# REGRAGUIahmed/DGViT-Depth-Goal-Guided-Vision-Transformer-

Hardware: AMD Instinct MI355X
Metric: depth frames/sec through DGViT fwd+bwd, batch 512x84x84 (higher is better)
Workload: dtype f32

## Files before the change

### dgvit-depth-goal-guided-vision-transformer-_amd/_lib.py

```python
import ctypes
import os
from ctypes import POINTER, Structure, c_char_p, c_float, c_int, c_longlong, c_ulonglong, c_void_p

_HERE = os.path.dirname(os.path.abspath(__file__))
LIB_PATH = os.path.join(_HERE, "libdgvit_hip.so")
DIAG_LIB_PATH = os.path.join(_HERE, "libdgvit_hip_diag.so")


class DgvitError(RuntimeError):
    pass


class dgvit_config(Structure):
    _fields_ = [("image_h", c_int), ("image_w", c_int), ("patch_h", c_int), ("patch_w", c_int), ("dim", c_int),
                ("depth", c_int), ("heads", c_int), ("dim_head", c_int), ("mlp_dim", c_int), ("pool_mean", c_int), ("flags", c_int)]


FLAG_DENSE_LAST_BLOCK = 1
FLAG_WGRAD_OVERLAP = 2
FLAG_LONG_SEQUENCE = 4
MAPS_GOAL = 0
MAPS_ALL = 1


# ... 79 lines not shown
    "dgvit_got_backward_bf16_ev": (_I, [_CFG, _TABLE, _P, _TABLE, _P, _P, _P, _P, _LL, _P, _LL, _I, _F, _ULL, _P, _P, POINTER(dgvit_grad_events)]),
    "dgvit_got_backward_bf16_v2": (_I, [_CFG, _TABLE, _P, _TABLE, _P, _P, _P, _P, _P, _LL, _P, _LL, _I, _F, _ULL, _P, _P]),
    "dgvit_got_backward_bf16_v2_ev": (_I, [_CFG, _TABLE, _P, _TABLE, _P, _P, _P, _P, _P, _LL, _P, _LL, _I, _F, _ULL, _P, _P,
                                           POINTER(dgvit_grad_events)]),
    "dgvit_wgrad_bf16_scratch_floats": (_LL, [_I, _I, _I]),
    "dgvit_wgrad_bf16": (_I, [_P, _P, _P, _P, _P, _LL, _I, _I, _I, _P]),
    "dgvit_cast_f32_bf16": (_I, [_P, _P, _LL, _P]),
    "dgvit_gemm_bf16": (_I, [_I, _P, _I, _P, _I, _P, _I, _I, _I, _I, _P, _P, _I, _P, _I, _P, _I, _P]),
    "dgvit_layernorm_forward_bf16": (_I, [_P, _P, _P, _P, _P, _P, _I, _I, _P]),
    "dgvit_attention_forward_bf16": (_I, [_P, _P, _P, _I, _I, _I, _I, _P]),
    "dgvit_got_forward_maps": (_I, [_CFG, _TABLE, _P, _P, _P, _P, _I, _P, _LL, _I, _F, _F, _ULL, _P, _P]),
    "dgvit_got_forward_maps_bf16": (_I, [_CFG, _TABLE, _P, _P, _P, _P, _P, _I, _P, _LL, _I, _F, _ULL, _P, _P]),
    "dgvit_attention_probs": (_I, [_P, _P, _P, _I, _I, _I, _I, _I, _P]),
    "dgvit_attention_probs_bf16": (_I, [_P, _P, _P, _I, _I, _I, _I, _I, _P]),
    "dgvit_attention_backward_bf16": (_I, [_P, _P, _P, _P, _P, _P, _I, _I, _I, _I, _P]),
    "dgvit_profile_start": (_I, [_I]),
    "dgvit_profile_stop": (_I, [POINTER(ctypes.c_double), POINTER(ctypes.c_double), POINTER(c_longlong)]),
    "dgvit_profile_sampling": (_I, [_I]),
    "dgvit_profile_totals": (_I, [POINTER(ctypes.c_double), POINTER(c_longlong)]),
}
DIAG_SIGNATURES = {
    "dgvit_set_gemm_tile": (None, [_I]),
    "dgvit_set_grouped_reduce": (None, [_I]),
    "dgvit_set_gemm_split": (None, [_I]),
    "dgvit_set_gemm_lds_pad": (None, [_I]),
    "dgvit_set_ln_fusion": (None, [_I]),
    "dgvit_set_conv_gather": (None, [_I]),
    "dgvit_set_gemm_diagnostics": (None, [_I]),
    "dgvit_set_gemm_persistent": (None, [_I, _I]),
    "dgvit_gemm_persistent_launches": (ctypes.c_longlong, []),
    "dgvit_set_gemm_stamps": (None, [_P, _I]),
    "dgvit_set_small_batch_path": (None, [_I, _I]),
    "dgvit_set_block_path": (None, [_I, _I]),
    "dgvit_set_block_stamps": (None, [_P]),
    "dgvit_set_block_stamp_layer": (None, [_I]),
    "dgvit_set_gelu_grad_store": (None, [_I]),
    "dgvit_set_block_fuse": (None, [_I]),
    "dgvit_set_gemm_bf16_tile": (None, [_I]),
    "dgvit_set_gemm_bf16_group_m": (None, [_I]),
    "dgvit_set_gemm_bf16_l2_budget_kb": (None, [_I]),
    "dgvit_set_attention_bwd_single_pass": (None, [_I]),
    "dgvit_set_attention_single_query": (None, [_I]),
    "dgvit_set_attention_bf16_long": (None, [_I]),
    "dgvit_set_gemm_wgrad_slice_major": (None, [_I]),
    "dgvit_attention_forward_queries": (_I, [_P, _P, _P, _I, _I, _I, _I, _I, _P]),
    "dgvit_attention_backward_queries": (_I, [_P, _P, _P, _P, _P, _I, _I, _I, _I, _I, _P]),
# ... 60 lines not shown
```

### dgvit-depth-goal-guided-vision-transformer-_amd/csrc/diag_api.hip

```cpp
#define DGVIT_KNOB_DEFINE
#include "../../include/dgvit_hip_diag.h"
#include "schedule.h"

#ifndef DGVIT_DIAG
#error "diag_api.hip belongs to the diagnostic library only (-DDGVIT_DIAG)"
#endif

long long g_gemm_persist_launches = 0;

extern "C" void dgvit_set_gemm_tile(int tile) { g_gemm_tile_hint = tile; }
extern "C" void dgvit_set_grouped_reduce(int on) { g_group_reduce = on ? 1 : 0; }
extern "C" void dgvit_set_conv_gather(int on) { g_conv_gather = on ? 1 : 0; }
extern "C" void dgvit_set_ln_fusion(int on) { g_ln_fusion = on ? 1 : 0; }
extern "C" void dgvit_set_gemm_split(int on) { g_gemm_split = on ? 1 : 0; }
extern "C" void dgvit_set_gemm_stamps(long long* stamps, int workgroups) {
  g_gemm_stamps = stamps;
  g_gemm_stamp_capacity = stamps ? workgroups : 0;
}
extern "C" long long dgvit_gemm_persistent_launches(void) { return g_gemm_persist_launches; }
extern "C" void dgvit_set_gemm_persistent(int mode, int workgroups) {
  g_gemm_persist = mode < 0 ? 0 : (mode > 2 ? 2 : mode);
  g_gemm_persist_grid = workgroups > 0 ? workgroups : 0;
}
extern "C" void dgvit_set_gemm_diagnostics(int on) { g_gemm_diag = on & 0x3FFFFF; }
extern "C" void dgvit_set_gemm_lds_pad(int bytes) { g_gemm_lds_pad = bytes > 0 ? bytes : 0; }
extern "C" void dgvit_set_small_batch_path(int on, int max_rows) {
  g_small_path = on ? 1 : 0;
  if (max_rows > 0) g_small_path_max_rows = max_rows;
}
extern "C" void dgvit_set_block_path(int on, int max_rows) {
  g_block_path = on < 0 ? 0 : (on > 2 ? 2 : on);
  g_block_path_max_rows = max_rows > 0 ? max_rows : g_block_path_max_rows_default;
}
extern "C" void dgvit_set_block_stamps(long long* stamps) { g_block_stamps = stamps; }
// ... 20 lines not shown
```

### dgvit-depth-goal-guided-vision-transformer-_amd/csrc/encoder.hip

```cpp
#include <mutex>

#include "schedule.h"

namespace {
struct Side {
  hipStream_t stream = nullptr;
  hipEvent_t ring[32];
  unsigned next = 0;
  bool ready = false;
};
Side g_side;
std::mutex g_side_mu;

int side_init() {
  std::lock_guard<std::mutex> lk(g_side_mu);
  if (g_side.ready) return DGVIT_OK;
  if (hipStreamCreateWithFlags(&g_side.stream, hipStreamNonBlocking) != hipSuccess)
    return dgvit_set_error(DGVIT_ERR_HIP, "cannot create the helper stream");
  for (auto& e : g_side.ring)
    if (hipEventCreateWithFlags(&e, hipEventDisableTiming) != hipSuccess)
      return dgvit_set_error(DGVIT_ERR_HIP, "cannot create helper events");
  g_side.ready = true;
  return DGVIT_OK;
}
int chain(hipStream_t from, hipStream_t to) {
  hipEvent_t e = g_side.ring[g_side.next++ % 32];
  if (hipEventRecord(e, from) != hipSuccess || hipStreamWaitEvent(to, e, 0) != hipSuccess)
    return dgvit_set_error(DGVIT_ERR_HIP, "event fork/join failed");
  return DGVIT_OK;
}
}
// ... 386 lines not shown
  f.maps_rows = rows;
  return got_forward(f, img, goal, feat, ws_floats, batch, keep);
}

namespace {

struct Bwd {
  const dgvit_config* cfg;
  Dims d;
  Ws w;
  Bs s;
  const float* const* params;
  float* const* grads;
  const float* ws;
  float* scratch;
  SplitBuf sk;
  float lkeep;
  bool ldrop;
  unsigned long long seed;
  const unsigned long long* seed_dev;
  hipStream_t st;
  hipStream_t sw;
  const dgvit_grad_events* events;
  LayerDrop site(int layer, int s) const { return LayerDrop{lkeep, drop_tag(layer, s), seed, seed_dev}; }
  int fork() const { return sw == st ? DGVIT_OK : chain(st, sw); }
  int join() const { return sw == st ? DGVIT_OK : chain(sw, st); }
};

int backward_layer(const Bwd& b, int i) {
  const Dims& d = b.d;
  const Ws& w = b.w;
  const Bs& s = b.s;
  const float* ws = b.ws;
  float* scratch = b.scratch;
  const bool ldrop = b.ldrop;
  hipStream_t st = b.st, sw = b.sw;
  const SplitBuf& sk = b.sk;
  const int T = (int)d.T;
  float* dx = scratch + s.dxa;
  float* dx2 = scratch + s.dxb;
  float* dln = scratch + s.dln;
  float* dqkv = scratch + s.dqkv;
  float* dao = scratch + s.dao;
  float* dh1 = scratch + s.dh1;
  float* slabs = scratch + s.slabs;
  const float* const* lp = b.params + P_L0 + DGVIT_PARAMS_PER_LAYER * i;
  float* const* lg = b.grads + P_L0 + DGVIT_PARAMS_PER_LAYER * i;
  const float* lb = ws + w.layer0 + w.layer_stride * i;
  const float* xin = i == 0 ? ws + w.x0 : ws + w.layer0 + w.layer_stride * (i - 1) + w.xout;
  const bool last = !dense_last_block(b.cfg) && !d.pool_mean && i == d.L - 1;
  const int tok = last ? d.B : T, rs = last ? d.N : 1;
  ReduceGroup grp;
  reduce_group_init(grp);
  ReduceGroup* gq = g_group_reduce ? &grp : nullptr;
  const float* dff = dx;
  if (ldrop) {
    TRY(drop_rows(dx, (long long)rs * d.D, scratch + s.dm3, (long long)rs * d.D, nullptr, 0, tok, d.D, rs, b.site(i, DROP_FF), st));
    dff = scratch + s.dm3;
  }
  TRY(b.fork());
  TRY(wgrad(dff, rs * d.D, lb + w.a1, d.M, lg[L_FC2W], lg[L_FC2B], d.D, d.M, tok, slabs + s.sl_fc2, s.n_fc2, sw, gq));
  {
    GemmParams p = gp(dff, rs * d.D, lp[L_FC2W], d.M, dh1, d.M, tok, d.M, d.D);
    p.aux = lb + w.h1; p.ldaux = d.M;
    sk.attach(p);
    TRY(gemm_f32(GEMM_NN, g_gelu_grad_store || ldrop ? EPI_DMUL : EPI_DGELU, p, 1, st));
  }
  TRY(b.fork());
  TRY(wgrad(dh1, d.M, lb + w.ln2, rs * d.D, lg[L_FC1W], lg[L_FC1B], d.M, d.D, tok, slabs + s.sl_fc1, s.n_fc1, sw, gq));
  {
    GemmParams p = gp(dh1, d.M, lp[L_FC1W], d.D, dln, rs * d.D, tok, d.D, d.M);
    sk.attach(p);
    TRY(gemm_f32(GEMM_NN, EPI_STORE, p, 1, st));
  }
  if (last) HIP_TRY(hipMemsetAsync(dx2, 0, sizeof(float) * d.T * d.D, st));
  TRY(layernorm_bwd(dln, lb + w.xmid, lb + w.mean2, lb + w.rstd2, lp[L_LN2W], dx, dx2, lg[L_LN2W], lg[L_LN2B], scratch + s.part_ln2, tok, d.D,
                    rs, st, gq));
  if (d.proj) {
    const float* dat = dx2;
    if (ldrop) {
      TRY(drop_rows(dx2, (long long)rs * d.D, scratch + s.dm1, (long long)rs * d.D, nullptr, 0, tok, d.D, rs, b.site(i, DROP_OUT), st));
      dat = scratch + s.dm1;
    }
    TRY(b.fork());
    TRY(wgrad(dat, rs * d.D, lb + w.ao, rs * d.I, lg[L_OUTW], lg[L_OUTB], d.D, d.I, tok, slabs + s.sl_out, s.n_out, sw, gq));
    GemmParams p = gp(dat, rs * d.D, lp[L_OUTW], d.I, dao, rs * d.I, tok, d.I, d.D);
    sk.attach(p);
    TRY(gemm_f32(GEMM_NN, EPI_STORE, p, 1, st));
  }
  const LayerDrop dr_attn = b.site(i, DROP_ATTN);
  if (d.tiled)
    TRY(attention_bwd_tiled(lb + w.qkv, lb + w.ao, d.proj ? dao : dx2, lb + w.lse, dqkv, scratch + s.delta, s.delta_floats, d.B, d.N, d.H,
                            d.dh, last ? 1 : d.N, st, ldrop ? &dr_attn : nullptr));
  else
    TRY(attention_bwd(lb + w.qkv, lb + w.ao, d.proj ? dao : dx2, lb + w.lse, dqkv, d.B, d.N, d.H, d.dh, last ? 1 : d.N, st,
                      ldrop ? &dr_attn : nullptr));
  TRY(b.fork());
  if (!last) {
    TRY(wgrad(dqkv, 3 * d.I, lb + w.ln1, d.D, lg[L_QKV], nullptr, 3 * d.I, d.D, T, slabs + s.sl_qkv, s.n_qkv, sw, gq));
    GemmParams p = gp(dqkv, 3 * d.I, lp[L_QKV], d.D, dln, d.D, T, d.D, 3 * d.I);
    sk.attach(p);
    TRY(gemm_f32(GEMM_NN, EPI_STORE, p, 1, st));
  } else {
    const long long nq_slabs = wgrad_scratch(d.I, d.D, tok);
    TRY(wgrad(dqkv, rs * 3 * d.I, lb + w.ln1, rs * d.D, lg[L_QKV], nullptr, d.I, d.D, tok, slabs + s.sl_qkv, nq_slabs, sw, gq));
    TRY(wgrad(dqkv + d.I, 3 * d.I, lb + w.ln1, d.D, lg[L_QKV] ? lg[L_QKV] + (long long)d.I * d.D : nullptr, nullptr, 2 * d.I, d.D, T,
              slabs + s.sl_qkv + nq_slabs, s.n_qkv - nq_slabs, sw, gq));
    GemmParams kv = gp(dqkv + d.I, 3 * d.I, lp[L_QKV] + (long long)d.I * d.D, d.D, dln, d.D, T, d.D, 2 * d.I);
    sk.attach(kv);
    TRY(gemm_f32(GEMM_NN, EPI_STORE, kv, 1, st));
    GemmParams q = gp(dqkv, rs * 3 * d.I, lp[L_QKV], d.D, dln, rs * d.D, tok, d.D, d.I);
    q.res = dln; q.ldr = rs * d.D;
    sk.attach(q);
    TRY(gemm_f32(GEMM_NN, EPI_STORE, q, 1, st));
  }
  TRY(b.join());
  TRY(layernorm_bwd(dln, xin, lb + w.mean1, lb + w.rstd1, lp[L_LN1W], dx2, dx, lg[L_LN1W], lg[L_LN1B], scratch + s.part_ln1, T, d.D, 1, st, gq));
  TRY(b.fork());
  TRY(reduce_group_flush(grp, sw));
  TRY(b.join());
  if (b.events) TRY(mark_ready(b.events->layer[i], st));
  return DGVIT_OK;
}

}

extern "C" int dgvit_got_backward(const dgvit_config* cfg, const float* const* params, float* const* grads, const float* dfeat,
                                  float* dgoal, const float* ws, long long ws_floats, float* scratch, long long scratch_floats,
                                  int batch, float keep, unsigned long long seed, const unsigned long long* seed_dev,
                                  void* stream) {
  return dgvit_got_backward_v2_ev(cfg, params, grads, dfeat, dgoal, ws, ws_floats, scratch, scratch_floats, batch, keep, 1.f, seed, seed_dev,
                                  stream, nullptr);
}

extern "C" int dgvit_got_backward_ev(const dgvit_config* cfg, const float* const* params, float* const* grads, const float* dfeat,
                                     float* dgoal, const float* ws, long long ws_floats, float* scratch, long long scratch_floats,
                                     int batch, float keep, unsigned long long seed, const unsigned long long* seed_dev,
                                     void* stream, const dgvit_grad_events* events) {
  return dgvit_got_backward_v2_ev(cfg, params, grads, dfeat, dgoal, ws, ws_floats, scratch, scratch_floats, batch, keep, 1.f, seed, seed_dev,
                                  stream, events);
}

extern "C" int dgvit_got_backward_v2(const dgvit_config* cfg, const float* const* params, float* const* grads, const float* dfeat,
// ... 5 lines not shown
}

extern "C" int dgvit_got_backward_v2_ev(const dgvit_config* cfg, const float* const* params, float* const* grads, const float* dfeat,
                                        float* dgoal, const float* ws, long long ws_floats, float* scratch, long long scratch_floats,
                                        int batch, float keep, float lkeep, unsigned long long seed, const unsigned long long* seed_dev,
                                        void* stream, const dgvit_grad_events* events) {
  return dgvit_got_backward_v3_ev(cfg, params, grads, dfeat, dgoal, nullptr, ws, ws_floats, scratch, scratch_floats, batch, keep, lkeep, seed,
                                  seed_dev, stream, events);
}

extern "C" int dgvit_got_backward_v3(const dgvit_config* cfg, const float* const* params, float* const* grads, const float* dfeat,
                                     float* dgoal, float* dimg, const float* ws, long long ws_floats, float* scratch, long long scratch_floats,
                                     int batch, float keep, float lkeep, unsigned long long seed, const unsigned long long* seed_dev,
                                     void* stream) {
  return dgvit_got_backward_v3_ev(cfg, params, grads, dfeat, dgoal, dimg, ws, ws_floats, scratch, scratch_floats, batch, keep, lkeep, seed,
                                  seed_dev, stream, nullptr);
}

extern "C" int dgvit_got_backward_v3_ev(const dgvit_config* cfg, const float* const* params, float* const* grads, const float* dfeat,
                                        float* dgoal, float* dimg, const float* ws, long long ws_floats, float* scratch, long long scratch_floats,
                                        int batch, float keep, float lkeep, unsigned long long seed, const unsigned long long* seed_dev,
                                        void* stream, const dgvit_grad_events* events) {
  hipStream_t st = (hipStream_t)stream;
  Bwd b = {cfg, {}, {}, {}, params, grads, ws, scratch, {}, lkeep, lkeep < 1.f, seed, seed_dev, st, st, events};
  const Dims& d = b.d;
  TRY(make_dims(cfg, batch, b.d));
  DGVIT_CHECK_ARG(params && grads && dfeat && ws && scratch, "dgvit_got_backward: null pointer");
  DGVIT_CHECK_ARG(keep > 0.f && keep <= 1.f, "dropout_keep must be in (0, 1]");
  DGVIT_CHECK_ARG(lkeep > 0.f && lkeep <= 1.f, "layer_dropout_keep must be in (0, 1]");
  TRY(check_events(events, cfg->depth));
  b.w = make_ws(d, 1);
  b.s = make_bs(d);
  const Ws& w = b.w;
  const Bs& s = b.s;
  if (ws_floats < w.total) return dgvit_set_error(DGVIT_ERR_WORKSPACE, "backward workspace %lld < %lld floats", ws_floats, w.total);
  if (scratch_floats < s.total) return dgvit_set_error(DGVIT_ERR_WORKSPACE, "backward scratch %lld < %lld floats", scratch_floats, s.total);
  const int np = P_L0 + DGVIT_PARAMS_PER_LAYER * d.L;
  for (int i = 0; i < np; ++i) DGVIT_CHECK_ARG(params[i] || no_projection_slot(d, i), "parameter %d is null", i);
  float* dx = scratch + s.dxa;
  float* dln = scratch + s.dln;
  float* part = scratch + s.part;

  if (s.sk_slab_floats > 0) {
    b.sk.counters = reinterpret_cast<int*>(scratch + s.sk_counters); b.sk.ncounters = (int)s.sk_ncounters;
    b.sk.slabs = scratch + s.sk_slabs; b.sk.slab_cap = s.sk_slab_floats;
    HIP_TRY(hipMemsetAsync(b.sk.counters, 0, sizeof(int) * s.sk_ncounters, st));
  }
  if (wgrad_overlap(cfg)) {
    TRY(side_init());
    b.sw = g_side.stream;
    TRY(chain(st, b.sw));
  }
  const float* xl = ws + w.layer0 + w.layer_stride * (d.L - 1) + w.xout;
  TRY(head_bwd(d, dfeat, xl, ws + w.pooled, params[P_RMS], grads[P_RMS], dx, dln, part, events, st));
  for (int i = d.L - 1; i >= 0; --i) TRY(backward_layer(b, i));
  return token_assembly_bwd(cfg, d, params, grads, dx, dgoal, dimg, dln, ws + w.patches, nullptr, nullptr, part, scratch + s.slabs,
                            s.slabs_floats, keep, seed, seed_dev, st);
}
```

### dgvit-depth-goal-guided-vision-transformer-_amd/csrc/kernels.h

```cpp
#pragma once
#include "common.h"

int layernorm_fwd(const float*, const float*, const float*, float*, float*, float*, int, int, float, int, hipStream_t);
int layernorm_bwd_blocks(int T);
int layernorm_bwd(const float*, const float*, const float*, const float*, const float*, const float*, float*, float*, float*,
                  float*, int, int, int, hipStream_t, ReduceGroup* grp = nullptr);
int rmsnorm_fwd(const float*, long long, const float*, float*, int, int, hipStream_t);
int rmsnorm_bwd_blocks(int B);
int rmsnorm_bwd(const float*, const float*, long long, const float*, float*, long long, float*, float*, int, int, hipStream_t);
int colsum_blocks(int T);
int colsum(const float*, long long, float*, float*, int, int, int, hipStream_t);
int attention_fwd(const float*, float*, float*, int, int, int, int, int, hipStream_t, const LayerDrop* drop = nullptr);
int attention_bwd(const float*, const float*, const float*, const float*, float*, int, int, int, int, int, hipStream_t,
                  const LayerDrop* drop = nullptr);
int attention_fwd_tiled(const float*, float*, float*, int, int, int, int, int, hipStream_t, const LayerDrop* drop = nullptr);
long long attention_bwd_tiled_scratch(int B, int N, int H);
int attention_bwd_tiled(const float*, const float*, const float*, const float*, float*, float*, long long, int, int, int, int, int,
                        hipStream_t, const LayerDrop* drop = nullptr);
int attention_probs(const float* qkv, const float* lse, float* probs, long long frame_stride, int B, int N, int H, int dh, int rows,
                    hipStream_t st);
int patchify(const float*, float*, int, int, int, int, int, hipStream_t);
int add_rows(const float*, long long, const float*, long long, float*, long long, long long, int, hipStream_t);
int goal_row(const float*, const float*, float*, int, int, int, hipStream_t);
int dropout_inplace(float*, long long, unsigned long long, const unsigned long long*, float, hipStream_t);
int drop_rows(const float* src, long long lds, float* dst, long long ldd, const float* res, long long ldr, long long rows, int width, int rs,
              const LayerDrop& drop, hipStream_t stream);
int relu_bwd(const float*, const float*, float*, long long, hipStream_t);
int adam_step(float*, const float*, float*, float*, long long, float, float, float, float, float, long long, const long long*,
              hipStream_t);
// ... 37 lines not shown
```

### dgvit-depth-goal-guided-vision-transformer-_amd/csrc/knobs.h

```cpp
#pragma once

#ifdef DGVIT_DIAG
#ifdef DGVIT_KNOB_DEFINE
#define DGVIT_KNOB(type, name, def) type name = def; constexpr type name##_default = def;
#else
#define DGVIT_KNOB(type, name, def) extern type name;
#endif
#define DGVIT_DIAG_ONLY(...) __VA_ARGS__
#define KNOB_IF(k) if (k)
#else
#define DGVIT_KNOB(type, name, def) static constexpr type name = def;
#define DGVIT_DIAG_ONLY(...)
#define KNOB_IF(k) if constexpr ((k) != 0)
#endif

DGVIT_KNOB(int, g_gemm_tile_hint, 0)
DGVIT_KNOB(int, g_gemm_split, 1)
DGVIT_KNOB(int, g_gemm_lds_pad, 0)
DGVIT_KNOB(int, g_gemm_persist, 0)
DGVIT_KNOB(int, g_gemm_persist_grid, 0)
DGVIT_KNOB(int, g_gemm_diag, 0)
DGVIT_KNOB(long long*, g_gemm_stamps, nullptr)
DGVIT_KNOB(int, g_gemm_stamp_capacity, 0)
DGVIT_KNOB(int, g_group_reduce, 1)
DGVIT_KNOB(int, g_ln_fusion, 1)
DGVIT_KNOB(int, g_conv_gather, 1)
DGVIT_KNOB(int, g_gelu_grad_store, 1)
DGVIT_KNOB(int, g_block_path, 1)
DGVIT_KNOB(int, g_block_fuse, 2)
DGVIT_KNOB(int, g_block_path_max_rows, 4160)
DGVIT_KNOB(long long*, g_block_stamps, nullptr)
DGVIT_KNOB(int, g_block_stamp_layer, -1)
DGVIT_KNOB(int, g_block_stamp_now, 1)
DGVIT_KNOB(int, g_small_path, 0)
DGVIT_KNOB(int, g_small_path_max_rows, 4160)
DGVIT_KNOB(int, g_gemm_bf16_tile_hint, 0)
DGVIT_KNOB(int, g_gemm_bf16_m16, 1)
DGVIT_KNOB(int, g_gemm_bf16_group_m, 8)
DGVIT_KNOB(int, g_gemm_bf16_l2_budget_kb, 2048)
DGVIT_KNOB(long long*, g_gemm_bf16_stamps, nullptr)
DGVIT_KNOB(int, g_attn_bwd64, 1)
DGVIT_KNOB(int, g_gemm_zfold, 1)
DGVIT_KNOB(int, g_attn_q1, 1)
DGVIT_KNOB(int, g_attn_bf16_long, 3)
#ifdef DGVIT_DIAG
extern long long g_gemm_persist_launches;
#endif
// ... 1 lines not shown
```

### dgvit-depth-goal-guided-vision-transformer-_amd/csrc/norm.hip

```cpp
#include "common.h"
#include "kernels.h"
#include "bf16.h"

namespace {

__device__ __forceinline__ float4 load4(const float* p) { return *reinterpret_cast<const float4*>(p); }
__device__ __forceinline__ float4 load4(const bf16_t* p) {
  const fx4 v = __builtin_convertvector(*reinterpret_cast<const bf16x4*>(p), fx4);
  return make_float4(v[0], v[1], v[2], v[3]);
}

__global__ void __launch_bounds__(256) layernorm_fwd_kernel(const float* __restrict__ x, const float* __restrict__ gamma,
                                                            const float* __restrict__ beta, float* __restrict__ y,
                                                            float* __restrict__ mean, float* __restrict__ rstd, int T, int D,
                                                            float eps, int rs) {
  const int lane = threadIdx.x & 63;
  const int row = blockIdx.x * 4 + (threadIdx.x >> 6);
  if (row >= T) return;
  const float* xr = x + (long long)row * rs * D;
  float s = 0.f;
  for (int c = lane * 4; c < D; c += 256) {
    const float4 v = *reinterpret_cast<const float4*>(xr + c);
    s += (v.x + v.y) + (v.z + v.w);
  }
// ... 8 lines not shown
  float* yr = y + (long long)row * rs * D;
  for (int c = lane * 4; c < D; c += 256) {
    const float4 v = *reinterpret_cast<const float4*>(xr + c);
    const float4 g = *reinterpret_cast<const float4*>(gamma + c);
    const float4 b = *reinterpret_cast<const float4*>(beta + c);
    float4 o;
    o.x = (v.x - mu) * rsd * g.x + b.x;
    o.y = (v.y - mu) * rsd * g.y + b.y;
    o.z = (v.z - mu) * rsd * g.z + b.z;
    o.w = (v.w - mu) * rsd * g.w + b.w;
    *reinterpret_cast<float4*>(yr + c) = o;
  }
  if (lane == 0) {
    mean[row] = mu;
    rstd[row] = rsd;
  }
}

template <int NCH, typename DYT>
__global__ void __launch_bounds__(256) layernorm_bwd_kernel(const DYT* __restrict__ dy, const float* __restrict__ x,
                                                            const float* __restrict__ mean, const float* __restrict__ rstd,
                                                            const float* __restrict__ gamma, const float* __restrict__ dres,
                                                            float* __restrict__ dx, bf16_t* __restrict__ dxb,
                                                            float* __restrict__ partial, int T, int D, int rs) {
  __shared__ float red[4][2][NCH * 256];
  const int lane = threadIdx.x & 63, wave = threadIdx.x >> 6;
  float4 ag[NCH], ab[NCH], gm[NCH];
#pragma unroll
  for (int i = 0; i < NCH; ++i) {
    ag[i] = make_float4(0.f, 0.f, 0.f, 0.f);
    ab[i] = ag[i];
    const int c = lane * 4 + i * 256;
    gm[i] = c < D ? *reinterpret_cast<const float4*>(gamma + c) : ag[i];
  }
  const float invD = 1.f / (float)D;
  for (int row = blockIdx.x * 4 + wave; row < T; row += gridDim.x * 4) {
    const long long off = (long long)row * rs * D;
    const float mu = mean[row], rsd = rstd[row];
    float4 g[NCH], xh[NCH];
    float s1 = 0.f, s2 = 0.f;
#pragma unroll
    for (int i = 0; i < NCH; ++i) {
      const int c = lane * 4 + i * 256;
      g[i] = make_float4(0.f, 0.f, 0.f, 0.f);
      xh[i] = g[i];
      if (c < D) {
        const float4 d = load4(dy + off + c);
        const float4 v = *reinterpret_cast<const float4*>(x + off + c);
        xh[i] = make_float4((v.x - mu) * rsd, (v.y - mu) * rsd, (v.z - mu) * rsd, (v.w - mu) * rsd);
        ag[i].x += d.x * xh[i].x; ag[i].y += d.y * xh[i].y; ag[i].z += d.z * xh[i].z; ag[i].w += d.w * xh[i].w;
        ab[i].x += d.x; ab[i].y += d.y; ab[i].z += d.z; ab[i].w += d.w;
        g[i] = make_float4(d.x * gm[i].x, d.y * gm[i].y, d.z * gm[i].z, d.w * gm[i].w);
        s1 += (g[i].x + g[i].y) + (g[i].z + g[i].w);
        s2 += (g[i].x * xh[i].x + g[i].y * xh[i].y) + (g[i].z * xh[i].z + g[i].w * xh[i].w);
      }
    }
    const float c1 = wave_sum(s1) * invD, c2 = wave_sum(s2) * invD;
#pragma unroll
    for (int i = 0; i < NCH; ++i) {
      const int c = lane * 4 + i * 256;
      if (c < D) {
        float4 o;
        o.x = rsd * (g[i].x - c1 - xh[i].x * c2);
        o.y = rsd * (g[i].y - c1 - xh[i].y * c2);
        o.z = rsd * (g[i].z - c1 - xh[i].z * c2);
        o.w = rsd * (g[i].w - c1 - xh[i].w * c2);
        if (dres) {
          const float4 r = *reinterpret_cast<const float4*>(dres + off + c);
          o.x += r.x; o.y += r.y; o.z += r.z; o.w += r.w;
        }
        *reinterpret_cast<float4*>(dx + off + c) = o;
        if (dxb) *reinterpret_cast<bf16x4*>(dxb + off + c) = __builtin_convertvector(fx4{o.x, o.y, o.z, o.w}, bf16x4);
      }
    }
  }
#pragma unroll
  for (int i = 0; i < NCH; ++i) {
    *reinterpret_cast<float4*>(&red[wave][0][i * 256 + lane * 4]) = ag[i];
    *reinterpret_cast<float4*>(&red[wave][1][i * 256 + lane * 4]) = ab[i];
  }
  __syncthreads();
  for (int c = threadIdx.x; c < 2 * NCH * 256; c += 256) {
    const int which = c / (NCH * 256), col = c % (NCH * 256);
    if (col < D) {
      const float s = ((red[0][which][col] + red[1][which][col]) + red[2][which][col]) + red[3][which][col];
      partial[((long long)blockIdx.x * 2 + which) * D + col] = s;
    }
  }
}

__global__ void __launch_bounds__(256) rmsnorm_fwd_kernel(const float* __restrict__ x, long long ldx, const float* __restrict__ g,
// ... 99 lines not shown
  DGVIT_CHECK_ARG(T > 0 && D > 0 && D % 4 == 0, "layernorm_fwd: D=%d must be a positive multiple of 4", D);
  DGVIT_CHECK_ARG(rs >= 1, "layernorm_fwd: bad row step");
  hipLaunchKernelGGL(layernorm_fwd_kernel, dim3((T + 3) / 4), dim3(256), 0, stream, x, gamma, beta, y, mean, rstd, T, D, eps, rs);
  DGVIT_CHECK_LAUNCH("layernorm_fwd");
  return DGVIT_OK;
}

int layernorm_bwd_blocks(int T) { return T < 2048 ? (T + 3) / 4 : (T < 16384 ? 512 : 2048); }
static int layernorm_bwd_blocks_f32(int T) { return T < 2048 ? (T + 3) / 4 : 512; }

static int ln_param_grads(const float* partial, float* dgamma, float* dbeta, int D, int nb, hipStream_t stream, ReduceGroup* grp) {
  ReduceGroup local;
  if (!grp) reduce_group_init(local);
  ReduceGroup& g = grp ? *grp : local;
  int rc = DGVIT_OK;
  if (dgamma && dbeta) rc = reduce_group_add(g, partial, dgamma, D, dbeta, 2ll * D, nb, 2ll * D, stream);
  else if (dgamma) rc = reduce_group_add(g, partial, dgamma, D, nullptr, D, nb, 2ll * D, stream);
  else if (dbeta) rc = reduce_group_add(g, partial + D, dbeta, D, nullptr, D, nb, 2ll * D, stream);
  if (rc || grp) return rc;
  return reduce_group_flush(local, stream);
}

int layernorm_bwd(const float* dy, const float* x, const float* mean, const float* rstd, const float* gamma, const float* dres,
                  float* dx, float* dgamma, float* dbeta, float* partial, int T, int D, int rs, hipStream_t stream, ReduceGroup* grp) {
  DGVIT_CHECK_ARG(dy && x && mean && rstd && gamma && dx && partial, "layernorm_bwd: null pointer");
  DGVIT_CHECK_ARG(T > 0 && D > 0 && D % 4 == 0 && D <= 1024, "layernorm_bwd: D=%d must be a multiple of 4, <= 1024", D);
  const int nb = layernorm_bwd_blocks_f32(T);
  const int nch = (D + 255) / 256;
#define LNB(NCH)                                                                                                              \
  hipLaunchKernelGGL((layernorm_bwd_kernel<NCH, float>), dim3(nb), dim3(256), 0, stream, dy, x, mean, rstd, gamma, dres, dx, \
                     (bf16_t*)nullptr, partial, T, D, rs)
  if (nch == 1) LNB(1);
  else if (nch == 2) LNB(2);
  else if (nch == 3) LNB(3);
  else LNB(4);
#undef LNB
  DGVIT_CHECK_LAUNCH("layernorm_bwd");
  return ln_param_grads(partial, dgamma, dbeta, D, nb, stream, grp);
}

int layernorm_bwd_bf16(const bf16_t* dy, const float* x, const float* mean, const float* rstd, const float* gamma, const float* dres,
                       float* dx, bf16_t* dxb, float* dgamma, float* dbeta, float* partial, int T, int D, int rs, hipStream_t stream) {
  DGVIT_CHECK_ARG(dy && x && mean && rstd && gamma && dx && partial, "layernorm_bwd_bf16: null pointer");
  DGVIT_CHECK_ARG(T > 0 && D > 0 && D % 4 == 0 && D <= 1024, "layernorm_bwd_bf16: D=%d must be a multiple of 4, <= 1024", D);
  const int nb = layernorm_bwd_blocks(T);
  const int nch = (D + 255) / 256;
  const int slot = profile_begin(PROF_OTHER, 0.0, stream);
#define LNB(NCH)                                                                                                              \
  hipLaunchKernelGGL((layernorm_bwd_kernel<NCH, bf16_t>), dim3(nb), dim3(256), 0, stream, dy, x, mean, rstd, gamma, dres, dx, dxb, \
                     partial, T, D, rs)
  if (nch == 1) LNB(1);
  else if (nch == 2) LNB(2);
  else if (nch == 3) LNB(3);
  else LNB(4);
#undef LNB
  profile_end(slot, stream);
  DGVIT_CHECK_LAUNCH("layernorm_bwd_bf16");
  return ln_param_grads(partial, dgamma, dbeta, D, nb, stream, nullptr);
}

int rmsnorm_fwd(const float* x, long long ldx, const float* g, float* y, int B, int D, hipStream_t stream) {
  DGVIT_CHECK_ARG(x && g && y && B > 0 && D > 0, "rmsnorm_fwd: bad arguments");
  hipLaunchKernelGGL(rmsnorm_fwd_kernel, dim3((B + 3) / 4), dim3(256), 0, stream, x, ldx, g, y, B, D);
  DGVIT_CHECK_LAUNCH("rmsnorm_fwd");
  return DGVIT_OK;
}

int rmsnorm_bwd_blocks(int B) { return B < 256 ? (B + 3) / 4 : 64; }

int rmsnorm_bwd(const float* dy, const float* x, long long ldx, const float* g, float* dx, long long lddx, float* dg,
                float* partial, int B, int D, hipStream_t stream) {
  DGVIT_CHECK_ARG(dy && x && g && dx && partial && B > 0 && D > 0 && D <= 4096, "rmsnorm_bwd: bad arguments");
  const int nb = rmsnorm_bwd_blocks(B);
// ... 18 lines not shown
```

### dgvit-depth-goal-guided-vision-transformer-_amd/csrc/schedule.h

```cpp
#pragma once
#include <algorithm>

#include "../../include/dgvit_hip.h"
#include "common.h"
#include "kernels.h"

#define TRY(expr)          \
  do {                     \
    int rc_ = (expr);      \
    if (rc_) return rc_;   \
  } while (0)

#define HIP_TRY(expr)                                                                        \
  do {                                                                                       \
    hipError_t e_ = (expr);                                                                  \
    if (e_ != hipSuccess) return dgvit_set_error(DGVIT_ERR_HIP, #expr ": %s", hipGetErrorString(e_)); \
  } while (0)

inline long long al4(long long n) { return (n + 3) & ~3ll; }

inline bool dense_last_block(const dgvit_config* c) { return (c->flags & DGVIT_FLAG_DENSE_LAST_BLOCK) != 0; }
inline bool wgrad_overlap(const dgvit_config* c) { return (c->flags & DGVIT_FLAG_WGRAD_OVERLAP) != 0; }
inline bool long_sequence(const dgvit_config* c) { return (c->flags & DGVIT_FLAG_LONG_SEQUENCE) != 0; }

// ... 111 lines not shown
  return j == L_OUTW || j == L_OUTB;
}

inline int check_events(const dgvit_grad_events* ev, int depth) {
  if (!ev) return DGVIT_OK;
  DGVIT_CHECK_ARG(ev->n_layers == depth, "dgvit_grad_events: n_layers %d != depth %d", ev->n_layers, depth);
  DGVIT_CHECK_ARG(ev->layer, "dgvit_grad_events: layer table is null");
  return DGVIT_OK;
}
inline int mark_ready(void* event, hipStream_t st) {
  if (event) HIP_TRY(hipEventRecord((hipEvent_t)event, st));
  return DGVIT_OK;
}

inline int pool_rmsnorm_fwd(const Dims& d, const float* x, float* pooled, const float* rms_g, float* feat, hipStream_t st) {
  if (d.pool_mean) {
    TRY(avgpool(x, pooled, d.B, d.N, d.D, st));
    return rmsnorm_fwd(pooled, d.D, rms_g, feat, d.B, d.D, st);
  }
  return rmsnorm_fwd(x, (long long)d.N * d.D, rms_g, feat, d.B, d.D, st);
}

inline int head_bwd(const Dims& d, const float* dfeat, const float* xl, const float* pooled, const float* rms_g, float* drms_g, float* dx,
                    float* dpool, float* part, const dgvit_grad_events* events, hipStream_t st) {
  if (d.pool_mean) {
    TRY(rmsnorm_bwd(dfeat, pooled, d.D, rms_g, dpool, d.D, drms_g, part, d.B, d.D, st));
    TRY(mean_bwd(dpool, dx, d.B, d.N, d.D, st));
  } else {
    HIP_TRY(hipMemsetAsync(dx, 0, sizeof(float) * d.T * d.D, st));
    TRY(rmsnorm_bwd(dfeat, xl, (long long)d.N * d.D, rms_g, dx, (long long)d.N * d.D, drms_g, part, d.B, d.D, st));
  }
  if (events) TRY(mark_ready(events->head, st));
  return DGVIT_OK;
}

inline int image_grad(const dgvit_config* c, const Dims& d, const float* dpatch, const float* wpe, float* dimg, hipStream_t st) {
  GemmParams p = gp(dpatch, d.D, wpe, d.pd, dimg, d.pd, d.B * d.P, d.pd, d.D);
  p.g_wi = c->image_w; p.g_hw = c->image_h * c->image_w; p.g_ph = c->patch_h; p.g_pw = c->patch_w;
  p.g_gw = c->image_w / c->patch_w; p.g_P = d.P;
  return gemm_f32(GEMM_NN, EPI_UNPATCH, p, 1, st);
}

inline int token_assembly_bwd(const dgvit_config* c, const Dims& d, const float* const* params, float* const* grads, float* dx, float* dgoal,
                              float* dimg, float* dpatch, const float* patches, const float* img, float* img32, float* part, float* slabs,
                              long long slab_floats, float keep, unsigned long long seed, const unsigned long long* seed_dev, hipStream_t st) {
  if (keep < 1.f) TRY(dropout_inplace(dx, d.T * d.D, seed, seed_dev, keep, st));
  if (dgoal)
    HIP_TRY(hipMemcpy2DAsync(dgoal, sizeof(float) * d.D, dx, sizeof(float) * d.N * d.D, sizeof(float) * d.D, d.B,
                             hipMemcpyDeviceToDevice, st));
  if (grads[P_POS]) TRY(colsum(dx, (long long)d.N * d.D, grads[P_POS], part, d.B, d.N * d.D, 0, st));
  const bool patch_grads = grads[P_PW] || grads[P_PB];
  if (!patch_grads && !dimg) return DGVIT_OK;
  HIP_TRY(hipMemcpy2DAsync(dpatch, sizeof(float) * d.P * d.D, dx + d.D, sizeof(float) * d.N * d.D, sizeof(float) * d.P * d.D, d.B,
                           hipMemcpyDeviceToDevice, st));
  if (patch_grads) {
    if (img) {
      TRY(patchify(img, img32, d.B, c->image_h, c->image_w, c->patch_h, c->patch_w, st));
      patches = img32;
    }
    TRY(wgrad(dpatch, d.D, patches, d.pd, grads[P_PW], grads[P_PB], d.D, d.pd, d.B * d.P, slabs, slab_floats, st));
  }
  if (dimg) TRY(image_grad(c, d, dpatch, params[P_PW], dimg, st));
  return DGVIT_OK;
}
```

### include/dgvit_hip_diag.h

```cpp
#ifndef DGVIT_HIP_DIAG_H
#define DGVIT_HIP_DIAG_H
#include "dgvit_hip.h"

#ifdef __cplusplus
extern "C" {
#endif
#pragma GCC visibility push(default)

void dgvit_set_gemm_tile(int tile);
void dgvit_set_grouped_reduce(int on);
void dgvit_set_gemm_split(int on);
void dgvit_set_ln_fusion(int on);
void dgvit_set_conv_gather(int on);
void dgvit_set_gemm_lds_pad(int bytes);
void dgvit_set_gemm_diagnostics(int bits);
void dgvit_set_gemm_persistent(int mode, int workgroups);
long long dgvit_gemm_persistent_launches(void);
void dgvit_set_gemm_stamps(long long* stamps, int workgroups);
void dgvit_set_small_batch_path(int on, int max_rows);
void dgvit_set_block_path(int on, int max_rows);
void dgvit_set_block_stamps(long long* stamps);
void dgvit_set_block_stamp_layer(int layer);
void dgvit_set_gelu_grad_store(int on);
void dgvit_set_block_fuse(int bits);
void dgvit_set_gemm_bf16_tile(int tile);
void dgvit_set_gemm_bf16_group_m(int rows);
void dgvit_set_gemm_bf16_l2_budget_kb(int kb);
void dgvit_set_attention_bwd_single_pass(int on);
void dgvit_set_attention_single_query(int on);
void dgvit_set_attention_bf16_long(int bits);
void dgvit_set_gemm_wgrad_slice_major(int on);
int dgvit_attention_forward_queries(const float* qkv, float* out, float* lse, int B, int N, int H, int dh, int nq, void* stream);
int dgvit_attention_backward_queries(const float* qkv, const float* out, const float* dout, const float* lse, float* dqkv, int B, int N, int H,
// ... 10 lines not shown
```

Before: 40690.

## Defer per-layer gradient reductions to a side stream during backward

```diff
diff --git a/dgvit-depth-goal-guided-vision-transformer-_amd/_lib.py b/dgvit-depth-goal-guided-vision-transformer-_amd/_lib.py
--- a/dgvit-depth-goal-guided-vision-transformer-_amd/_lib.py
+++ b/dgvit-depth-goal-guided-vision-transformer-_amd/_lib.py
@@ -125,6 +125,8 @@
 DIAG_SIGNATURES = {
     "dgvit_set_gemm_tile": (None, [_I]),
     "dgvit_set_grouped_reduce": (None, [_I]),
+    "dgvit_set_side_reductions": (None, [_I]),
+    "dgvit_got_backward_scratch_layout": (_I, [_CFG, _I, POINTER(c_longlong), _I]),
     "dgvit_set_gemm_split": (None, [_I]),
     "dgvit_set_gemm_lds_pad": (None, [_I]),
     "dgvit_set_ln_fusion": (None, [_I]),
diff --git a/dgvit-depth-goal-guided-vision-transformer-_amd/csrc/diag_api.hip b/dgvit-depth-goal-guided-vision-transformer-_amd/csrc/diag_api.hip
--- a/dgvit-depth-goal-guided-vision-transformer-_amd/csrc/diag_api.hip
+++ b/dgvit-depth-goal-guided-vision-transformer-_amd/csrc/diag_api.hip
@@ -10,6 +10,7 @@
 
 extern "C" void dgvit_set_gemm_tile(int tile) { g_gemm_tile_hint = tile; }
 extern "C" void dgvit_set_grouped_reduce(int on) { g_group_reduce = on ? 1 : 0; }
+extern "C" void dgvit_set_side_reductions(int on) { g_side_reductions = on ? 1 : 0; }
 extern "C" void dgvit_set_conv_gather(int on) { g_conv_gather = on ? 1 : 0; }
 extern "C" void dgvit_set_ln_fusion(int on) { g_ln_fusion = on ? 1 : 0; }
 extern "C" void dgvit_set_gemm_split(int on) { g_gemm_split = on ? 1 : 0; }
diff --git a/dgvit-depth-goal-guided-vision-transformer-_amd/csrc/encoder.hip b/dgvit-depth-goal-guided-vision-transformer-_amd/csrc/encoder.hip
--- a/dgvit-depth-goal-guided-vision-transformer-_amd/csrc/encoder.hip
+++ b/dgvit-depth-goal-guided-vision-transformer-_amd/csrc/encoder.hip
@@ -1,12 +1,18 @@
+#include <atomic>
 #include <mutex>
+#include <utility>
+#include <vector>
 
 #include "schedule.h"
+#ifdef DGVIT_DIAG
+#include "../../include/dgvit_hip_diag.h"
+#endif
 
 namespace {
 struct Side {
   hipStream_t stream = nullptr;
   hipEvent_t ring[32];
-  unsigned next = 0;
+  std::atomic<unsigned> next{0};
   bool ready = false;
 };
 Side g_side;
@@ -439,12 +445,25 @@
   hipStream_t st;
   hipStream_t sw;
   const dgvit_grad_events* events;
+  hipStream_t ss;
+  bool side;
+  ReduceGroup pending;
+  int pending_layer;
   LayerDrop site(int layer, int s) const { return LayerDrop{lkeep, drop_tag(layer, s), seed, seed_dev}; }
-  int fork() const { return sw == st ? DGVIT_OK : chain(st, sw); }
-  int join() const { return sw == st ? DGVIT_OK : chain(sw, st); }
+  int fork(hipStream_t to) const { return to == st ? DGVIT_OK : chain(st, to); }
+  int join(hipStream_t from) const { return from == st ? DGVIT_OK : chain(from, st); }
 };
 
-int backward_layer(const Bwd& b, int i) {
+int flush_pending(Bwd& b) {
+  if (b.pending_layer < 0) return DGVIT_OK;
+  TRY(b.fork(b.ss));
+  TRY(reduce_group_flush(b.pending, b.ss));
+  if (b.events) TRY(mark_ready(b.events->layer[b.pending_layer], b.ss));
+  b.pending_layer = -1;
+  return DGVIT_OK;
+}
+
+int backward_layer(Bwd& b, int i) {
   const Dims& d = b.d;
   const Ws& w = b.w;
   const Bs& s = b.s;
@@ -454,6 +473,8 @@
   hipStream_t st = b.st, sw = b.sw;
   const SplitBuf& sk = b.sk;
   const int T = (int)d.T;
+  const bool waited = b.side && b.pending_layer >= 0;
+  if (waited) TRY(flush_pending(b));
   float* dx = scratch + s.dxa;
   float* dx2 = scratch + s.dxb;
   float* dln = scratch + s.dln;
@@ -461,13 +482,16 @@
   float* dao = scratch + s.dao;
   float* dh1 = scratch + s.dh1;
   float* slabs = scratch + s.slabs;
+  float* part_ln2 = scratch + s.part_ln2;
+  float* part_ln1 = scratch + s.part_ln1;
   const float* const* lp = b.params + P_L0 + DGVIT_PARAMS_PER_LAYER * i;
   float* const* lg = b.grads + P_L0 + DGVIT_PARAMS_PER_LAYER * i;
   const float* lb = ws + w.layer0 + w.layer_stride * i;
   const float* xin = i == 0 ? ws + w.x0 : ws + w.layer0 + w.layer_stride * (i - 1) + w.xout;
   const bool last = !dense_last_block(b.cfg) && !d.pool_mean && i == d.L - 1;
   const int tok = last ? d.B : T, rs = last ? d.N : 1;
-  ReduceGroup grp;
+  hipStream_t sl = last ? b.ss : sw;
+  ReduceGroup& grp = b.pending;
   reduce_group_init(grp);
   ReduceGroup* gq = g_group_reduce ? &grp : nullptr;
   const float* dff = dx;
@@ -475,32 +499,42 @@
     TRY(drop_rows(dx, (long long)rs * d.D, scratch + s.dm3, (long long)rs * d.D, nullptr, 0, tok, d.D, rs, b.site(i, DROP_FF), st));
     dff = scratch + s.dm3;
   }
-  TRY(b.fork());
-  TRY(wgrad(dff, rs * d.D, lb + w.a1, d.M, lg[L_FC2W], lg[L_FC2B], d.D, d.M, tok, slabs + s.sl_fc2, s.n_fc2, sw, gq));
-  {
+  auto fc2_wgrad = [&]() -> int {
+    TRY(b.fork(sl));
+    return wgrad(dff, rs * d.D, lb + w.a1, d.M, lg[L_FC2W], lg[L_FC2B], d.D, d.M, tok, slabs + s.sl_fc2, s.n_fc2, sl, gq);
+  };
+  auto fc2_dgrad = [&]() -> int {
     GemmParams p = gp(dff, rs * d.D, lp[L_FC2W], d.M, dh1, d.M, tok, d.M, d.D);
     p.aux = lb + w.h1; p.ldaux = d.M;
     sk.attach(p);
-    TRY(gemm_f32(GEMM_NN, g_gelu_grad_store || ldrop ? EPI_DMUL : EPI_DGELU, p, 1, st));
-  }
-  TRY(b.fork());
-  TRY(wgrad(dh1, d.M, lb + w.ln2, rs * d.D, lg[L_FC1W], lg[L_FC1B], d.M, d.D, tok, slabs + s.sl_fc1, s.n_fc1, sw, gq));
+    return gemm_f32(GEMM_NN, g_gelu_grad_store || ldrop ? EPI_DMUL : EPI_DGELU, p, 1, st);
+  };
+  if (b.side) {
+    TRY(fc2_dgrad());
+    if (waited) TRY(b.join(b.ss));
+    TRY(fc2_wgrad());
+  } else {
+    TRY(fc2_wgrad());
+    TRY(fc2_dgrad());
+  }
+  TRY(b.fork(sl));
+  TRY(wgrad(dh1, d.M, lb + w.ln2, rs * d.D, lg[L_FC1W], lg[L_FC1B], d.M, d.D, tok, slabs + s.sl_fc1, s.n_fc1, sl, gq));
   {
     GemmParams p = gp(dh1, d.M, lp[L_FC1W], d.D, dln, rs * d.D, tok, d.D, d.M);
     sk.attach(p);
     TRY(gemm_f32(GEMM_NN, EPI_STORE, p, 1, st));
   }
-  if (last) HIP_TRY(hipMemsetAsync(dx2, 0, sizeof(float) * d.T * d.D, st));
-  TRY(layernorm_bwd(dln, lb + w.xmid, lb + w.mean2, lb + w.rstd2, lp[L_LN2W], dx, dx2, lg[L_LN2W], lg[L_LN2B], scratch + s.part_ln2, tok, d.D,
-                    rs, st, gq));
+  const bool sparse_res = last && b.side;
+  if (last && !sparse_res) HIP_TRY(hipMemsetAsync(dx2, 0, sizeof(float) * d.T * d.D, st));
+  TRY(layernorm_bwd(dln, lb + w.xmid, lb + w.mean2, lb + w.rstd2, lp[L_LN2W], dx, dx2, lg[L_LN2W], lg[L_LN2B], part_ln2, tok, d.D, rs, st, gq));
   if (d.proj) {
     const float* dat = dx2;
     if (ldrop) {
       TRY(drop_rows(dx2, (long long)rs * d.D, scratch + s.dm1, (long long)rs * d.D, nullptr, 0, tok, d.D, rs, b.site(i, DROP_OUT), st));
       dat = scratch + s.dm1;
     }
-    TRY(b.fork());
-    TRY(wgrad(dat, rs * d.D, lb + w.ao, rs * d.I, lg[L_OUTW], lg[L_OUTB], d.D, d.I, tok, slabs + s.sl_out, s.n_out, sw, gq));
+    TRY(b.fork(sl));
+    TRY(wgrad(dat, rs * d.D, lb + w.ao, rs * d.I, lg[L_OUTW], lg[L_OUTB], d.D, d.I, tok, slabs + s.sl_out, s.n_out, sl, gq));
     GemmParams p = gp(dat, rs * d.D, lp[L_OUTW], d.I, dao, rs * d.I, tok, d.I, d.D);
     sk.attach(p);
     TRY(gemm_f32(GEMM_NN, EPI_STORE, p, 1, st));
@@ -512,7 +546,8 @@
   else
     TRY(attention_bwd(lb + w.qkv, lb + w.ao, d.proj ? dao : dx2, lb + w.lse, dqkv, d.B, d.N, d.H, d.dh, last ? 1 : d.N, st,
                       ldrop ? &dr_attn : nullptr));
-  TRY(b.fork());
+  TRY(b.fork(sl));
+  if (sw != sl) TRY(b.fork(sw));
   if (!last) {
     TRY(wgrad(dqkv, 3 * d.I, lb + w.ln1, d.D, lg[L_QKV], nullptr, 3 * d.I, d.D, T, slabs + s.sl_qkv, s.n_qkv, sw, gq));
     GemmParams p = gp(dqkv, 3 * d.I, lp[L_QKV], d.D, dln, d.D, T, d.D, 3 * d.I);
@@ -520,7 +555,7 @@
     TRY(gemm_f32(GEMM_NN, EPI_STORE, p, 1, st));
   } else {
     const long long nq_slabs = wgrad_scratch(d.I, d.D, tok);
-    TRY(wgrad(dqkv, rs * 3 * d.I, lb + w.ln1, rs * d.D, lg[L_QKV], nullptr, d.I, d.D, tok, slabs + s.sl_qkv, nq_slabs, sw, gq));
+    TRY(wgrad(dqkv, rs * 3 * d.I, lb + w.ln1, rs * d.D, lg[L_QKV], nullptr, d.I, d.D, tok, slabs + s.sl_qkv, nq_slabs, sl, gq));
     TRY(wgrad(dqkv + d.I, 3 * d.I, lb + w.ln1, d.D, lg[L_QKV] ? lg[L_QKV] + (long long)d.I * d.D : nullptr, nullptr, 2 * d.I, d.D, T,
               slabs + s.sl_qkv + nq_slabs, s.n_qkv - nq_slabs, sw, gq));
     GemmParams kv = gp(dqkv + d.I, 3 * d.I, lp[L_QKV] + (long long)d.I * d.D, d.D, dln, d.D, T, d.D, 2 * d.I);
@@ -531,11 +566,17 @@
     sk.attach(q);
     TRY(gemm_f32(GEMM_NN, EPI_STORE, q, 1, st));
   }
-  TRY(b.join());
-  TRY(layernorm_bwd(dln, xin, lb + w.mean1, lb + w.rstd1, lp[L_LN1W], dx2, dx, lg[L_LN1W], lg[L_LN1B], scratch + s.part_ln1, T, d.D, 1, st, gq));
-  TRY(b.fork());
+  TRY(b.join(sw));
+  if (sl != sw) TRY(b.join(sl));
+  TRY(layernorm_bwd(dln, xin, lb + w.mean1, lb + w.rstd1, lp[L_LN1W], dx2, dx, lg[L_LN1W], lg[L_LN1B], part_ln1, T, d.D, 1, st, gq,
+                    sparse_res ? d.N : 1));
+  if (b.side) {
+    b.pending_layer = i;
+    return DGVIT_OK;
+  }
+  TRY(b.fork(sw));
   TRY(reduce_group_flush(grp, sw));
-  TRY(b.join());
+  TRY(b.join(sw));
   if (b.events) TRY(mark_ready(b.events->layer[i], st));
   return DGVIT_OK;
 }
@@ -587,7 +628,7 @@
                                         int batch, float keep, float lkeep, unsigned long long seed, const unsigned long long* seed_dev,
                                         void* stream, const dgvit_grad_events* events) {
   hipStream_t st = (hipStream_t)stream;
-  Bwd b = {cfg, {}, {}, {}, params, grads, ws, scratch, {}, lkeep, lkeep < 1.f, seed, seed_dev, st, st, events};
+  Bwd b = {cfg, {}, {}, {}, params, grads, ws, scratch, {}, lkeep, lkeep < 1.f, seed, seed_dev, st, st, events, st, g_side_reductions != 0, {}, -1};
   const Dims& d = b.d;
   TRY(make_dims(cfg, batch, b.d));
   DGVIT_CHECK_ARG(params && grads && dfeat && ws && scratch, "dgvit_got_backward: null pointer");
@@ -611,14 +652,52 @@
     b.sk.slabs = scratch + s.sk_slabs; b.sk.slab_cap = s.sk_slab_floats;
     HIP_TRY(hipMemsetAsync(b.sk.counters, 0, sizeof(int) * s.sk_ncounters, st));
   }
-  if (wgrad_overlap(cfg)) {
+  if (wgrad_overlap(cfg) || b.side) {
     TRY(side_init());
-    b.sw = g_side.stream;
-    TRY(chain(st, b.sw));
+    if (wgrad_overlap(cfg)) b.sw = g_side.stream;
+    b.ss = g_side.stream;
+    TRY(chain(st, g_side.stream));
   }
   const float* xl = ws + w.layer0 + w.layer_stride * (d.L - 1) + w.xout;
-  TRY(head_bwd(d, dfeat, xl, ws + w.pooled, params[P_RMS], grads[P_RMS], dx, dln, part, events, st));
+  if (!b.side) {
+    TRY(head_bwd(d, dfeat, xl, ws + w.pooled, params[P_RMS], grads[P_RMS], dx, dln, part, events, st));
+    for (int i = d.L - 1; i >= 0; --i) TRY(backward_layer(b, i));
+    return token_assembly_bwd(cfg, d, params, grads, dx, dgoal, dimg, dln, ws + w.patches, nullptr, nullptr, part, scratch + s.slabs,
+                              s.slabs_floats, keep, seed, seed_dev, st);
+  }
+  const bool token0_last = !dense_last_block(cfg) && !d.pool_mean;
+  TRY(head_bwd(d, dfeat, xl, ws + w.pooled, params[P_RMS], nullptr, dx, dln, part, nullptr, st, !token0_last));
+  TRY(b.fork(b.ss));
+  if (grads[P_RMS]) TRY(reduce_slabs(part, grads[P_RMS], d.D, rmsnorm_bwd_blocks(d.B), d.D, b.ss));
+  if (events) TRY(mark_ready(events->head, b.ss));
   for (int i = d.L - 1; i >= 0; --i) TRY(backward_layer(b, i));
-  return token_assembly_bwd(cfg, d, params, grads, dx, dgoal, dimg, dln, ws + w.patches, nullptr, nullptr, part, scratch + s.slabs,
-                            s.slabs_floats, keep, seed, seed_dev, st);
-}
+  TRY(b.join(b.ss));
+  TRY(flush_pending(b));
+  hipEvent_t done = g_side.ring[g_side.next++ % 32];
+  HIP_TRY(hipEventRecord(done, b.ss));
+  TRY(token_assembly_bwd(cfg, d, params, grads, dx, dgoal, dimg, dln, ws + w.patches, nullptr, nullptr, part, scratch + s.slabs,
+                         s.slabs_floats, keep, seed, seed_dev, st, done));
+  HIP_TRY(hipStreamWaitEvent(st, done, 0));
+  return DGVIT_OK;
+}
+
+#ifdef DGVIT_DIAG
+extern "C" int dgvit_got_backward_scratch_layout(const dgvit_config* cfg, int batch, long long* regions, int capacity) {
+  Dims d;
+  if (make_dims(cfg, batch, d)) return -1;
+  const Bs s = make_bs(d);
+  const long long td = al4(d.T * d.D), lnp = al4((long long)layernorm_bwd_blocks((int)d.T) * 2 * d.D);
+  std::vector<std::pair<long long, long long>> r = {
+      {s.dxa, td}, {s.dxb, td}, {s.dln, td}, {s.dqkv, al4(d.T * 3 * d.I)}, {s.dao, al4(d.T * d.I)}, {s.dh1, al4(d.T * d.M)},
+      {s.dm1, td}, {s.dm3, td}, {s.part, s.part_ln2 - s.part}, {s.part_ln2, lnp}, {s.part_ln1, lnp},
+      {s.slabs + s.sl_fc2, s.n_fc2}, {s.slabs + s.sl_fc1, s.n_fc1}, {s.slabs + s.sl_out, s.n_out}, {s.slabs + s.sl_qkv, s.n_qkv}};
+  r.push_back({s.sk_counters, al4(s.sk_ncounters)});
+  r.push_back({s.sk_slabs, al4(s.sk_slab_floats)});
+  r.push_back({s.delta, al4(s.delta_floats)});
+  for (int i = 0; i < (int)r.size() && i < capacity; ++i) {
+    regions[2 * i] = r[i].first;
+    regions[2 * i + 1] = r[i].second;
+  }
+  return (int)r.size();
+}
+#endif
diff --git a/dgvit-depth-goal-guided-vision-transformer-_amd/csrc/kernels.h b/dgvit-depth-goal-guided-vision-transformer-_amd/csrc/kernels.h
--- a/dgvit-depth-goal-guided-vision-transformer-_amd/csrc/kernels.h
+++ b/dgvit-depth-goal-guided-vision-transformer-_amd/csrc/kernels.h
@@ -4,7 +4,7 @@
 int layernorm_fwd(const float*, const float*, const float*, float*, float*, float*, int, int, float, int, hipStream_t);
 int layernorm_bwd_blocks(int T);
 int layernorm_bwd(const float*, const float*, const float*, const float*, const float*, const float*, float*, float*, float*,
-                  float*, int, int, int, hipStream_t, ReduceGroup* grp = nullptr);
+                  float*, int, int, int, hipStream_t, ReduceGroup* grp = nullptr, int res_rs = 1);
 int rmsnorm_fwd(const float*, long long, const float*, float*, int, int, hipStream_t);
 int rmsnorm_bwd_blocks(int B);
 int rmsnorm_bwd(const float*, const float*, long long, const float*, float*, long long, float*, float*, int, int, hipStream_t);
diff --git a/dgvit-depth-goal-guided-vision-transformer-_amd/csrc/knobs.h b/dgvit-depth-goal-guided-vision-transformer-_amd/csrc/knobs.h
--- a/dgvit-depth-goal-guided-vision-transformer-_amd/csrc/knobs.h
+++ b/dgvit-depth-goal-guided-vision-transformer-_amd/csrc/knobs.h
@@ -23,6 +23,7 @@
 DGVIT_KNOB(long long*, g_gemm_stamps, nullptr)
 DGVIT_KNOB(int, g_gemm_stamp_capacity, 0)
 DGVIT_KNOB(int, g_group_reduce, 1)
+DGVIT_KNOB(int, g_side_reductions, 1)
 DGVIT_KNOB(int, g_ln_fusion, 1)
 DGVIT_KNOB(int, g_conv_gather, 1)
 DGVIT_KNOB(int, g_gelu_grad_store, 1)
diff --git a/dgvit-depth-goal-guided-vision-transformer-_amd/csrc/norm.hip b/dgvit-depth-goal-guided-vision-transformer-_amd/csrc/norm.hip
--- a/dgvit-depth-goal-guided-vision-transformer-_amd/csrc/norm.hip
+++ b/dgvit-depth-goal-guided-vision-transformer-_amd/csrc/norm.hip
@@ -54,7 +54,7 @@
                                                             const float* __restrict__ mean, const float* __restrict__ rstd,
                                                             const float* __restrict__ gamma, const float* __restrict__ dres,
                                                             float* __restrict__ dx, bf16_t* __restrict__ dxb,
-                                                            float* __restrict__ partial, int T, int D, int rs) {
+                                                            float* __restrict__ partial, int T, int D, int rs, int res_rs) {
   __shared__ float red[4][2][NCH * 256];
   const int lane = threadIdx.x & 63, wave = threadIdx.x >> 6;
   float4 ag[NCH], ab[NCH], gm[NCH];
@@ -98,7 +98,8 @@
         o.z = rsd * (g[i].z - c1 - xh[i].z * c2);
         o.w = rsd * (g[i].w - c1 - xh[i].w * c2);
         if (dres) {
-          const float4 r = *reinterpret_cast<const float4*>(dres + off + c);
+          float4 r = make_float4(0.f, 0.f, 0.f, 0.f);
+          if (res_rs <= 1 || row % res_rs == 0) r = *reinterpret_cast<const float4*>(dres + off + c);
           o.x += r.x; o.y += r.y; o.z += r.z; o.w += r.w;
         }
         *reinterpret_cast<float4*>(dx + off + c) = o;
@@ -244,14 +245,16 @@
 }
 
 int layernorm_bwd(const float* dy, const float* x, const float* mean, const float* rstd, const float* gamma, const float* dres,
-                  float* dx, float* dgamma, float* dbeta, float* partial, int T, int D, int rs, hipStream_t stream, ReduceGroup* grp) {
+                  float* dx, float* dgamma, float* dbeta, float* partial, int T, int D, int rs, hipStream_t stream, ReduceGroup* grp,
+                  int res_rs) {
   DGVIT_CHECK_ARG(dy && x && mean && rstd && gamma && dx && partial, "layernorm_bwd: null pointer");
+  DGVIT_CHECK_ARG(res_rs >= 1, "layernorm_bwd: bad residual row step");
   DGVIT_CHECK_ARG(T > 0 && D > 0 && D % 4 == 0 && D <= 1024, "layernorm_bwd: D=%d must be a multiple of 4, <= 1024", D);
   const int nb = layernorm_bwd_blocks_f32(T);
   const int nch = (D + 255) / 256;
 #define LNB(NCH)                                                                                                              \
   hipLaunchKernelGGL((layernorm_bwd_kernel<NCH, float>), dim3(nb), dim3(256), 0, stream, dy, x, mean, rstd, gamma, dres, dx, \
-                     (bf16_t*)nullptr, partial, T, D, rs)
+                     (bf16_t*)nullptr, partial, T, D, rs, res_rs)
   if (nch == 1) LNB(1);
   else if (nch == 2) LNB(2);
   else if (nch == 3) LNB(3);
@@ -270,7 +273,7 @@
   const int slot = profile_begin(PROF_OTHER, 0.0, stream);
 #define LNB(NCH)                                                                                                              \
   hipLaunchKernelGGL((layernorm_bwd_kernel<NCH, bf16_t>), dim3(nb), dim3(256), 0, stream, dy, x, mean, rstd, gamma, dres, dx, dxb, \
-                     partial, T, D, rs)
+                     partial, T, D, rs, 1)
   if (nch == 1) LNB(1);
   else if (nch == 2) LNB(2);
   else if (nch == 3) LNB(3);
diff --git a/dgvit-depth-goal-guided-vision-transformer-_amd/csrc/schedule.h b/dgvit-depth-goal-guided-vision-transformer-_amd/csrc/schedule.h
--- a/dgvit-depth-goal-guided-vision-transformer-_amd/csrc/schedule.h
+++ b/dgvit-depth-goal-guided-vision-transformer-_amd/csrc/schedule.h
@@ -157,12 +157,12 @@
 }
 
 inline int head_bwd(const Dims& d, const float* dfeat, const float* xl, const float* pooled, const float* rms_g, float* drms_g, float* dx,
-                    float* dpool, float* part, const dgvit_grad_events* events, hipStream_t st) {
+                    float* dpool, float* part, const dgvit_grad_events* events, hipStream_t st, bool zero_rows = true) {
   if (d.pool_mean) {
     TRY(rmsnorm_bwd(dfeat, pooled, d.D, rms_g, dpool, d.D, drms_g, part, d.B, d.D, st));
     TRY(mean_bwd(dpool, dx, d.B, d.N, d.D, st));
   } else {
-    HIP_TRY(hipMemsetAsync(dx, 0, sizeof(float) * d.T * d.D, st));
+    if (zero_rows) HIP_TRY(hipMemsetAsync(dx, 0, sizeof(float) * d.T * d.D, st));
     TRY(rmsnorm_bwd(dfeat, xl, (long long)d.N * d.D, rms_g, dx, (long long)d.N * d.D, drms_g, part, d.B, d.D, st));
   }
   if (events) TRY(mark_ready(events->head, st));
@@ -178,7 +178,8 @@
 
 inline int token_assembly_bwd(const dgvit_config* c, const Dims& d, const float* const* params, float* const* grads, float* dx, float* dgoal,
                               float* dimg, float* dpatch, const float* patches, const float* img, float* img32, float* part, float* slabs,
-                              long long slab_floats, float keep, unsigned long long seed, const unsigned long long* seed_dev, hipStream_t st) {
+                              long long slab_floats, float keep, unsigned long long seed, const unsigned long long* seed_dev, hipStream_t st,
+                              hipEvent_t slabs_ready = nullptr) {
   if (keep < 1.f) TRY(dropout_inplace(dx, d.T * d.D, seed, seed_dev, keep, st));
   if (dgoal)
     HIP_TRY(hipMemcpy2DAsync(dgoal, sizeof(float) * d.D, dx, sizeof(float) * d.N * d.D, sizeof(float) * d.D, d.B,
@@ -193,6 +194,7 @@
       TRY(patchify(img, img32, d.B, c->image_h, c->image_w, c->patch_h, c->patch_w, st));
       patches = img32;
     }
+    if (slabs_ready) HIP_TRY(hipStreamWaitEvent(st, slabs_ready, 0));
     TRY(wgrad(dpatch, d.D, patches, d.pd, grads[P_PW], grads[P_PB], d.D, d.pd, d.B * d.P, slabs, slab_floats, st));
   }
   if (dimg) TRY(image_grad(c, d, dpatch, params[P_PW], dimg, st));
diff --git a/include/dgvit_hip_diag.h b/include/dgvit_hip_diag.h
--- a/include/dgvit_hip_diag.h
+++ b/include/dgvit_hip_diag.h
@@ -9,6 +9,8 @@
 
 void dgvit_set_gemm_tile(int tile);
 void dgvit_set_grouped_reduce(int on);
+void dgvit_set_side_reductions(int on);
+int dgvit_got_backward_scratch_layout(const dgvit_config* cfg, int batch, long long* regions, int capacity);
 void dgvit_set_gemm_split(int on);
 void dgvit_set_ln_fusion(int on);
 void dgvit_set_conv_gather(int on);
```

After: 40640. No clear change (-0.1%).
